# pydata/sparse

Hardware: AMD Instinct MI355X
Metric: GCXS x dense SpMM throughput (GFLOP/s) (higher is better)
Workload: dtype f32; 1 GPU; GCXS(CSR) 1000000x10000 @ 0.01 (100000000 nnz, int32 idx) in 1 nnz-balanced row block(s) x dense 10000x128 fp32; world_size=1, rows_rank0=1000000, idx_dtype=int32, parallelism=row-block x1, mul_add=fma, nan_warning=deferred, prewarm_products=40, default_settings=NAN_WARNING="sync" (verdict read inside every product), kernel=spmm_tiled (cached block stream)

## Files before the change

sparse_amd/csrc/build.py:

```python
import concurrent.futures as cf
import glob
import os
import shutil
import subprocess
import sys

HERE = os.path.dirname(os.path.abspath(__file__))
PKG = os.path.dirname(HERE)
OUT_DIR = os.path.join(PKG, "_lib")
OBJ_DIR = os.path.join(OUT_DIR, "obj")
LIB = os.path.join(OUT_DIR, "libsparse_amd.so")
ARCH = "gfx950"
CXXFLAGS = [
    f"--offload-arch={ARCH}", "-O3", "-std=c++17", "-fPIC", "-ffp-contract=off",
    "-fno-gpu-rdc", "-Wall", "-Wno-unused-function", "-Wno-unused-variable",
]


def _hipcc():
    for c in (os.environ.get("HIPCC"), shutil.which("hipcc"), "/opt/rocm/bin/hipcc"):
        if c and os.path.exists(c):
            return c
    raise RuntimeError("hipcc not found (need ROCm to build libsparse_amd.so)")


def sources():
    return sorted(glob.glob(os.path.join(HERE, "*.hip")))


def _deps():
    return sorted(glob.glob(os.path.join(HERE, "*.h"))) + sorted(glob.glob(os.path.join(HERE, "*.inc"))) + [
        os.path.join(os.path.dirname(PKG), "include", "sparse_amd.h"), os.path.abspath(__file__)]


def is_stale():
    if not os.path.exists(LIB):
        return True
    t = os.path.getmtime(LIB)
    return any(os.path.getmtime(p) > t for p in sources() + _deps())


def _own_deps(src, obj):
    dep = obj[:-2] + ".d"
    if not os.path.exists(dep):
        return _deps()
    words = open(dep).read().replace("\\\n", " ").split()
    files = [w for w in words[1:] if not w.startswith("/opt/") and not w.startswith("/usr/")]
    if any(not os.path.exists(f) for f in files):
        return _deps()
    return files + [os.path.abspath(__file__)]


NO_SPILL = {"spmm_tiled.hip": "spmm_tiled_kernel"}


def _spills(remarks, needle):
    out, name, sg = [], None, 0
    for ln in remarks.splitlines():
        if "Function Name:" in ln:
            name = ln.split("Function Name:")[1].split()[0]
        elif "SGPRs Spill:" in ln:
            sg = int(ln.split("SGPRs Spill:")[1].split()[0])
        elif "VGPRs Spill:" in ln and name is not None:
            vg = int(ln.split("VGPRs Spill:")[1].split()[0])
            if needle in name and (sg or vg):
                out.append((name, sg, vg))
    return out


def _compile(src, force):
    obj = os.path.join(OBJ_DIR, os.path.basename(src)[:-4] + ".o")
    newest = max(os.path.getmtime(p) for p in [src] + _own_deps(src, obj))
    if not force and os.path.exists(obj) and os.path.getmtime(obj) >= newest:
        return obj, ""
    needle = NO_SPILL.get(os.path.basename(src))
    extra = ["-Rpass-analysis=kernel-resource-usage"] if needle else []
    cmd = [_hipcc(), *CXXFLAGS, *extra, "-MD", "-MF", obj[:-2] + ".d", "-c", src, "-o", obj]
    r = subprocess.run(cmd, capture_output=True, text=True)
    if r.returncode != 0:
        raise RuntimeError(f"hipcc failed for {src}:\n{' '.join(cmd)}\n{r.stdout}\n{r.stderr}")
    if needle:
        bad = _spills(r.stderr, needle)
        if bad:
            os.remove(obj)
            raise RuntimeError(f"{os.path.basename(src)}: the compiler spilled registers in " +
                               ", ".join(f"{n[:60]} ({s} SGPR, {v} VGPR)" for n, s, v in bad[:4]) +
                               " - refused (see NO_SPILL in sparse_amd/csrc/build.py)")
        return obj, "\n".join(ln for ln in r.stderr.splitlines() if "-Rpass-analysis" not in ln and "remark:" not in ln)
    return obj, r.stderr


def build(force=False, verbose=False, jobs=None):
    if not force and not is_stale():
        return LIB
    os.makedirs(OBJ_DIR, exist_ok=True)
    srcs = sources()
    jobs = jobs or min(len(srcs), os.cpu_count() or 1)
    with cf.ThreadPoolExecutor(max_workers=jobs) as ex:
        results = list(ex.map(lambda s: _compile(s, force), srcs))
    objs = [o for o, _ in results]
    if verbose:
        for _, w in results:
            if w.strip():
                print(w, file=sys.stderr)
    cmd = [_hipcc(), f"--offload-arch={ARCH}", "-shared", "-fPIC", "-o", LIB + ".tmp", *objs]
    r = subprocess.run(cmd, capture_output=True, text=True)
    if r.returncode != 0:
        raise RuntimeError(f"link failed:\n{' '.join(cmd)}\n{r.stdout}\n{r.stderr}")
    os.replace(LIB + ".tmp", LIB)
    return LIB


if __name__ == "__main__":
    p = build(force="--force" in sys.argv, verbose=True)
    print(p)
```

sparse_amd/csrc/spmm_tiled.hip:

```cpp
#include "common.h"
#include "spmm_tiled_asm.inc"
#include <stdlib.h>
#include <mutex>
#include <set>

namespace spamd {

constexpr int TL_RG = TL_ASM_RG;
constexpr int TL_WAVES = TL_ASM_WAVES;
#ifndef SPAMD_TL_EXPERIMENTAL
static_assert(TL_RG == 35 && TL_WAVES == 16, "experimental tiled-SpMM geometry: build with -DSPAMD_TL_EXPERIMENTAL");
#endif
constexpr int TL_KB = TL_ASM_KB;
constexpr int TL_NBUF = 2;
__host__ __device__ constexpr int tl_d0(int lc, int lr) { return ((lc >> 1) << 11) | ((lc & 1) << 9) | (2 + 2 * lr); }
constexpr int TL_BLOCK_INTS = 16;

template <typename T>
struct TlFmt;
template <>
struct TlFmt<float> {
  static constexpr int EPB = 8, PANEL = 128;
  __device__ static void put(int* stream, int64_t entry, int d0, float v) {
    int* b = stream + (entry / EPB) * TL_BLOCK_INTS + (entry % EPB) * 2;
    typedef int int2v __attribute__((ext_vector_type(2)));
    int2v e;
    e.x = d0;
    e.y = __builtin_bit_cast(int, v);
    *reinterpret_cast<int2v*>(b) = e;
  }
};
template <>
struct TlFmt<double> {
  static constexpr int EPB = 5, PANEL = 64;
  __device__ static void put(int* stream, int64_t entry, int d0, double v) {
    int* b = stream + (entry / EPB) * TL_BLOCK_INTS;
    const int slot = (int)(entry % EPB);
    const long long bits = __builtin_bit_cast(long long, v);
    b[slot] = d0;
    if (slot == 0) b[5] = 0;
    *reinterpret_cast<long long*>(b + 6 + 2 * slot) = bits;
  }
};
typedef int tl_srd_t __attribute__((ext_vector_type(4)));
constexpr int TL_TILE = TL_KB * 512;
constexpr int TL_LDS = TL_NBUF * TL_TILE;
constexpr int TL_DMA_PER_TILE = TL_TILE / 16 / (TL_WAVES * 64);
static_assert(TL_LDS <= 160 * 1024 && TL_KB % (2 * TL_WAVES) == 0 && TL_DMA_PER_TILE == TL_ASM_DMA_PER_TILE,
              "tile geometry is baked into gen_tiled_asm.py");
constexpr int TL_SLACK_BLOCKS = 68;

#define GRID_STRIDE(i, n)                                                          \
  for (int64_t i = (int64_t)blockIdx.x * blockDim.x + threadIdx.x; i < (n);        \
       i += (int64_t)gridDim.x * blockDim.x)

__global__ void __launch_bounds__(256) tl_keys_kernel(const int64_t* __restrict__ rc_keys, int64_t nnz, int64_t K,
                                                      int64_t ntiles, int64_t* __restrict__ out) {
  GRID_STRIDE(i, nnz) {
    const int64_t k = rc_keys[i];
    const int64_t row = k / K, col = k - row * K;
    const int64_t g = row / TL_RG, lr = row - g * TL_RG, t = col / TL_KB, lc = col - t * TL_KB;
    out[i] = ((g * ntiles + t) * TL_RG + lr) * TL_KB + lc;
  }
}

__global__ void __launch_bounds__(256) tl_seg_start_kernel(const int64_t* __restrict__ keys, int64_t nnz,
                                                           int64_t nseg, int64_t* __restrict__ seg_start) {
  GRID_STRIDE(i, nnz + 1) {
    const int64_t hi = i < nnz ? keys[i] / (TL_RG * TL_KB) : nseg;
    const int64_t lo = i > 0 ? keys[i - 1] / (TL_RG * TL_KB) + 1 : 0;
    for (int64_t s = lo; s <= hi; ++s) seg_start[s] = i;
  }
}

__global__ void __launch_bounds__(256) tl_blocks_kernel(const int64_t* __restrict__ seg_start, int64_t nseg, int epb,
                                                        int64_t* __restrict__ nblk) {
  GRID_STRIDE(s, nseg + 1) {
    nblk[s] = s < nseg ? (seg_start[s + 1] - seg_start[s] + epb - 1) / epb : 0;
  }
}

template <typename T>
__global__ void __launch_bounds__(256) tl_pack_kernel(const int64_t* __restrict__ keys, const T* __restrict__ vals,
                                                      int64_t nnz, const int64_t* __restrict__ seg_start,
                                                      const int64_t* __restrict__ blk_off, int* __restrict__ stream) {
  GRID_STRIDE(i, nnz) {
    const int64_t k = keys[i];
    const int64_t lc = k % TL_KB, r1 = k / TL_KB, lr = r1 % TL_RG, s = r1 / TL_RG;
    const int64_t dst = blk_off[s] * TlFmt<T>::EPB + (i - seg_start[s]);
    TlFmt<T>::put(stream, dst, tl_d0((int)lc, (int)lr), vals[i]);
  }
}

constexpr int TL_DIRECT_MAX_TILES = 256;

template <typename I>
__device__ __forceinline__ int tl_row_of(const int64_t* rs, int64_t e) {
  static_assert(TL_RG <= 128, "seven bisection steps");
  int lo = 0, hi = TL_RG;
#pragma unroll
  for (int it = 0; it < (TL_RG <= 64 ? 6 : 7); ++it) {
    const int mid = (lo + hi) >> 1;
    if (hi - lo > 1) {
      if (rs[mid] <= e) lo = mid; else hi = mid;
    }
  }
  return lo;
}

template <typename I>
__global__ void __launch_bounds__(256) tl_count_kernel(int64_t M, int ntiles, int epb, const I* __restrict__ indices,
                                                       const I* __restrict__ indptr, int64_t* __restrict__ nblk,
                                                       int* __restrict__ flags) {
  __shared__ int cnt[TL_DIRECT_MAX_TILES];
  __shared__ int64_t rs[TL_RG + 1];
  const int tid = threadIdx.x;
  const int64_t r0 = (int64_t)blockIdx.x * TL_RG;
  if (tid <= TL_RG) {
    const int64_t r = r0 + tid;
    rs[tid] = (int64_t)indptr[r < M ? r : M];
  }
  for (int t = tid; t < ntiles; t += 256) cnt[t] = 0;
  __syncthreads();
  const int64_t e0 = rs[0], e1 = rs[TL_RG];
  bool bad = false;
  for (int64_t e = e0 + tid; e < e1; e += 256) {
    const int64_t c = (int64_t)indices[e];
    atomicAdd(&cnt[(int)(c / TL_KB)], 1);
    if (e > e0 && (int64_t)indices[e - 1] > c && rs[tl_row_of<I>(rs, e)] != e) bad = true;
  }
  if (bad) flags[0] = 1;
  __syncthreads();
  for (int t = tid; t < ntiles; t += 256) nblk[(int64_t)blockIdx.x * ntiles + t] = (cnt[t] + epb - 1) / epb;
}

template <typename I, typename T>
__global__ void __launch_bounds__(256) tl_fill_kernel(int64_t M, int ntiles, const T* __restrict__ vals,
                                                      const I* __restrict__ indices, const I* __restrict__ indptr,
                                                      const int64_t* __restrict__ blk_off, int* __restrict__ stream) {
  extern __shared__ int tl_fill_lds[];
  __shared__ int64_t rs[TL_RG + 1];
  int* const before = tl_fill_lds;
  int* const runstart = before + TL_RG * ntiles;
  const int tid = threadIdx.x;
  const int64_t r0 = (int64_t)blockIdx.x * TL_RG;
  if (tid <= TL_RG) {
    const int64_t r = r0 + tid;
    rs[tid] = (int64_t)indptr[r < M ? r : M];
  }
  for (int i = tid; i < TL_RG * ntiles; i += 256) before[i] = 0;
  __syncthreads();
  const int64_t e0 = rs[0], e1 = rs[TL_RG];
  for (int64_t e = e0 + tid; e < e1; e += 256) {
    const int t = (int)((int64_t)indices[e] / TL_KB);
// ... 23 lines not shown

__host__ __device__ inline int64_t tl_group_first_block(int64_t e0, int64_t g, int64_t ntiles, int64_t epb) {
  return (e0 + g * ntiles * (epb - 1) + epb - 1) / epb;
}

template <typename I, typename T, bool MAPPED>
__global__ void __launch_bounds__(256) tl_inspect_kernel(int64_t M, int ntiles, int64_t groups, const T* __restrict__ vals,
                                                         const I* __restrict__ indices, const I* __restrict__ indptr,
                                                         unsigned long long* __restrict__ state, int* __restrict__ blk_off,
                                                         int* __restrict__ stream, const int* __restrict__ rowmap,
                                                         const int64_t* __restrict__ vstart) {
  extern __shared__ int tl_fill_lds[];
  __shared__ __attribute__((aligned(16))) int64_t rsab[2 * (TL_RG + 1)];
  __shared__ int wtot[5];
  __shared__ int group_bad;
  constexpr int EPB = TlFmt<T>::EPB;
  int* const before = tl_fill_lds;
  int* const runstart = before + TL_RG * ntiles;
  int* const loff = runstart + TL_RG * ntiles;
  const int tid = threadIdx.x;
  const int64_t g = blockIdx.x;
  const int64_t r0 = g * TL_RG;
  if (tid < TL_RG) {
    if constexpr (MAPPED) {
      const int r = rowmap[r0 + tid];
      rsab[2 * (tid)] = r >= 0 ? (int64_t)indptr[r] : 0;
      rsab[2 * (tid) + 1] = r >= 0 ? (int64_t)indptr[r + 1] : 0;
    } else {
      const int64_t r = r0 + tid;
      rsab[2 * (tid)] = (int64_t)indptr[r < M ? r : M];
      rsab[2 * (tid) + 1] = (int64_t)indptr[r + 1 < M ? r + 1 : M];
    }
  }
  for (int i = tid; i < TL_RG * ntiles; i += 256) before[i] = 0;
  if (tid == 0) group_bad = 0;
  __syncthreads();
  const int64_t e0 = MAPPED ? vstart[g] : rsab[2 * (0)], e1 = MAPPED ? vstart[g + 1] : rsab[2 * (TL_RG - 1) + 1];
  bool bad = false;
  constexpr int RPW = (TL_RG + 3) / 4;
  constexpr int TL_PRE = 2;
  const int wv = tid >> 6, lane = tid & 63;
  unsigned cpre[RPW][TL_PRE];
  T vpre[RPW][TL_PRE];
#pragma unroll
  for (int i = 0; i < RPW; ++i) {
    const int lr = wv + 4 * i;
    const int64_t ra = lr < TL_RG ? rsab[2 * (lr)] : 0, rb = lr < TL_RG ? rsab[2 * (lr) + 1] : 0;
#pragma unroll
    for (int p = 0; p < TL_PRE; ++p) {
      const int64_t e = ra + lane + 64 * p;
      cpre[i][p] = e < rb ? (unsigned)indices[e] : 0xffffffffu;
      vpre[i][p] = e < rb ? vals[e] : T(0);
    }
  }
  auto count_one = [&](int lr, int64_t ra, int64_t e, unsigned c, unsigned cp, bool row_start) {
    const int t = (int)(c / (unsigned)TL_KB);
    atomicAdd(&before[lr * ntiles + t], 1);
    if (!row_start && cp > c) bad = true;
    if (row_start || (int)(cp / (unsigned)TL_KB) != t) runstart[lr * ntiles + t] = (int)(e - (MAPPED ? ra : e0));
  };
#pragma unroll
  for (int i = 0; i < RPW; ++i) {
    const int lr = wv + 4 * i;
    if (lr >= TL_RG) break;
    const int64_t ra = rsab[2 * (lr)], rb = rsab[2 * (lr) + 1];
#pragma unroll
    for (int p = 0; p < TL_PRE; ++p) {
      const int64_t e = ra + lane + 64 * p;
      const unsigned c = cpre[i][p];
      unsigned cp = (unsigned)__shfl_up((int)c, 1, 64);
      if (p > 0) {
        const unsigned last = (unsigned)__builtin_amdgcn_readlane((int)cpre[i][p > 0 ? p - 1 : 0], 63);
        if (lane == 0) cp = last;
      }
      if (e < rb) count_one(lr, ra, e, c, cp, p == 0 && lane == 0);
    }
    for (int64_t e = ra + lane + 64 * TL_PRE; e < rb; e += 64)
      count_one(lr, ra, e, (unsigned)indices[e], (unsigned)indices[e - 1], false);
  }
  if (bad) {
    atomicOr(&state[0], 1ull);
    group_bad = 1;
  }
  __syncthreads();
  int nb = 0, cnt_t = 0;
  for (int t = tid; t < ntiles; t += 256) {
    int c[TL_RG];
#pragma unroll
    for (int lr = 0; lr < TL_RG; ++lr) c[lr] = before[lr * ntiles + t];
    int run = 0;
#pragma unroll
    for (int lr = 0; lr < TL_RG; ++lr) {
      before[lr * ntiles + t] = run;
      run += c[lr];
    }
    cnt_t = run;
    nb = (run + EPB - 1) / EPB;
  }
  const int wid = wv;
  int x = nb;
#pragma unroll
  for (int d = 1; d < 64; d <<= 1) {
    const int y = __shfl_up(x, d, 64);
    if (lane >= d) x += y;
  }
  if (lane == 63) wtot[wid] = x;
  __syncthreads();
  int woff = 0;
  for (int w = 0; w < wid; ++w) woff += wtot[w];
  const int gtotal = wtot[0] + wtot[1] + wtot[2] + wtot[3];
  const int my_off = woff + x - nb;
  const int64_t goff = tl_group_first_block(e0, g, ntiles, EPB);
  const int64_t gnext = tl_group_first_block(e1, g + 1, ntiles, EPB);
  if (tid < ntiles) loff[tid] = my_off;
  __syncthreads();
  if (tid < ntiles) blk_off[g * (ntiles + 1) + tid] = (int)(goff + my_off);
  if (tid == 0) blk_off[g * (ntiles + 1) + ntiles] = (int)(goff + gtotal);
  for (int64_t i = (goff + gtotal) * TL_BLOCK_INTS + tid; i < gnext * TL_BLOCK_INTS; i += 256) stream[i] = 0;
  if (group_bad) {
    for (int64_t i = goff * TL_BLOCK_INTS + tid; i < (goff + gtotal) * TL_BLOCK_INTS; i += 256) stream[i] = 0;
    return;
  }
  auto fill_one = [&](int lr, int64_t ra, int64_t e, unsigned c, T v) {
    const int t = (int)(c / (unsigned)TL_KB);
    const int lc = (int)(c - (unsigned)t * (unsigned)TL_KB);
    const int64_t dst = (goff + loff[t]) * EPB + before[lr * ntiles + t] + ((int)(e - (MAPPED ? ra : e0)) - runstart[lr * ntiles + t]);
    TlFmt<T>::put(stream, dst, tl_d0(lc, lr), v);
  };
#pragma unroll
  for (int i = 0; i < RPW; ++i) {
    const int lr = wv + 4 * i;
    if (lr >= TL_RG) break;
    const int64_t ra = rsab[2 * (lr)], rb = rsab[2 * (lr) + 1];
#pragma unroll
    for (int p = 0; p < TL_PRE; ++p) {
      const int64_t e = ra + lane + 64 * p;
      if (e < rb) fill_one(lr, ra, e, cpre[i][p], vpre[i][p]);
    }
    for (int64_t e = ra + lane + 64 * TL_PRE; e < rb; e += 64) fill_one(lr, ra, e, (unsigned)indices[e], vals[e]);
  }
  if (tid < ntiles) {
    const int64_t first = (goff + my_off) * EPB;
    for (int i = cnt_t; i < nb * EPB; ++i) TlFmt<T>::put(stream, first + i, 0, T(0));
  }
}

__device__ __forceinline__ void tl_dma16(unsigned lds_base, const void* src) {
  asm volatile("s_mov_b32 m0, %0\n\ts_nop 0\n\tglobal_load_lds_dwordx4 %1, off"
               :
               : "s"(lds_base), "v"(src)
               : "memory", "m0");
}

template <int MODE>
__device__ __forceinline__ void tl_phases(const int* stream, int t0, int te, int o0, int o1, int o2, int offreg, int obase,
                                          int ntiles, int nfull, int toff, int mask, unsigned m0wave,
                                          unsigned row_step, int voff, tl_srd_t srd, unsigned& soff) {
  const int lane = threadIdx.x & 63;
  const unsigned blo = (unsigned)((uintptr_t)stream & 0xffffffffu), bhi = (unsigned)((uintptr_t)stream >> 32);
  const int lane8 = lane * 8;
#define TL_PHASES_OPERANDS                                                                                        \
  [soff] "+s"(soff)                                                                                               \
  : [blo] "s"(blo), [bhi] "s"(bhi), [t0] "s"(t0), [te] "s"(te), [o0] "s"(o0), [o1] "s"(o1), [o2] "s"(o2),         \
    [obase] "s"(obase), [ntiles] "s"(ntiles), [nfull] "s"(nfull), [m0wave] "s"(m0wave), [step] "s"(row_step),      \
    [toff] "v"(toff), [lane8] "v"(lane8), [mask] "v"(mask), [offreg] "v"(offreg), [voff] "v"(voff), [srd] "s"(srd)  \
  : "memory", "m0", "scc", "vcc", TL_CLOB_SGPR, TL_CLOB_TMP, TL_CLOB_ACC
  if (MODE == 6)
    asm volatile(TL_ASM_PHASES_I32 : TL_PHASES_OPERANDS);
  else if (MODE == 4)
    asm volatile(TL_ASM_PHASES_F64 : TL_PHASES_OPERANDS);
  else if (MODE == 5)
    asm volatile(TL_ASM_PHASES_F64_EXACT : TL_PHASES_OPERANDS);
  else if (MODE == 3)
    asm volatile(TL_ASM_PHASES_EXACT : TL_PHASES_OPERANDS);
  else if (MODE == 1)
    asm volatile(TL_ASM_PHASES_NOFMA : TL_PHASES_OPERANDS);
  else if (MODE == 2)
    asm volatile(TL_ASM_PHASES_NOLDS : TL_PHASES_OPERANDS);
  else
    asm volatile(TL_ASM_PHASES : TL_PHASES_OPERANDS);
#undef TL_PHASES_OPERANDS
}

__device__ __forceinline__ void tl_block_map(unsigned L, int npanels, int nblocks, int& bx, int& by) {
  const unsigned pin = npanels > 1 ? 2u : 1u;
  const unsigned per_chunk = (unsigned)((nblocks + 7) / 8) * 8u * pin;
  const unsigned chunk = L / per_chunk, l = L % per_chunk;
  const unsigned seq = l >> 3;
  by = uniform((int)(chunk * pin + seq % pin));
  bx = uniform((int)((seq / pin) * 8u + (l & 7u)));
}

template <int DBG, int MODE, typename T>
__global__ void __launch_bounds__(TL_WAVES * 64) __attribute__((amdgpu_num_vgpr(TL_ASM_COMP)))
spmm_tiled_kernel(int64_t M, int64_t K, int ntiles, int touch_lines, const int* __restrict__ stream,
                  const int* __restrict__ blk_off, const T* __restrict__ b, int64_t ldb,
                  T* __restrict__ out, int64_t ldo, int last_cols, int npanels, int nblocks, const int* __restrict__ rowmap) {
  constexpr int PANEL = TlFmt<T>::PANEL;
  constexpr int CPL = PANEL / 64;
  extern __shared__ __attribute__((aligned(16))) char lds[];
  const int tid = threadIdx.x;
  const int lane = tid & 63;
  const int wv = uniform(tid >> 6);
  int bx, by;
  tl_block_map(blockIdx.x, npanels, nblocks, bx, by);
  if (bx >= nblocks || by >= npanels) return;
  const int g = bx * TL_WAVES + wv;
  b += (int64_t)by * PANEL;
  out += (int64_t)by * PANEL;

  asm volatile(TL_ASM_ZERO ::: "memory", TL_CLOB_ACC);

  const int nfull = DBG == 2 ? 0 : (int)(K / TL_KB);
  const unsigned row_step = (unsigned)((2 * TL_WAVES) * ldb * (int64_t)sizeof(T));
  const unsigned m0wave = (unsigned)wv * 2048u;
  const uint64_t bbase = (uint64_t)(uintptr_t)b;
  tl_srd_t srd;
  srd[0] = (int)(bbase & 0xffffffffu);
  srd[1] = (int)((bbase >> 32) & 0xffffu);
  srd[2] = (int)0xffffffffu;
  srd[3] = 0x00020000;
  const int voff = (int)((int64_t)(tid >> 5) * ldb * (int64_t)sizeof(T)) + (tid & 31) * 16;
  unsigned soff = 0;
  auto issue_partial = [&](int t) {
#pragma unroll
    for (int i = 0; i < TL_DMA_PER_TILE; ++i) {
      const int e = (i * (TL_WAVES * 64) + tid) * 16;
      int64_t r = (int64_t)t * TL_KB + (e >> 9);
      if (r >= K) r = K - 1;
      tl_dma16(((unsigned)(i * TL_WAVES + wv) * 2u + (unsigned)(t & 1)) * 1024u,
               reinterpret_cast<const char*>(b + r * ldb) + (e & 511));
    }
  };
  const bool has_partial = DBG != 2 && (int64_t)nfull * TL_KB < K;

  if (nfull > 0)
    asm volatile(TL_ASM_TILE0 : [soff] "+s"(soff) : [m0wave] "s"(m0wave), [step] "s"(row_step), [voff] "v"(voff), [srd] "s"(srd) : "memory", "m0", "scc", "vcc", "s89");
  else if (has_partial)
    issue_partial(0);
  asm volatile("s_waitcnt vmcnt(0)" ::: "memory");
  __syncthreads();

  const int* const myoff = blk_off + (int64_t)g * (ntiles + (touch_lines >> 16));
  touch_lines &= 0xffff;
  const int toff = (lane < touch_lines ? lane : touch_lines - 1) * 64;
  int t = 0;
  while (t < ntiles) {
    const int obase = t;
    const int q = obase + lane;
    int offreg = myoff[q < ntiles ? q : ntiles];
    asm volatile("" : "+v"(offreg));
    int te = obase + 61 < ntiles ? obase + 61 : ntiles;
    if (has_partial && t < nfull - 1 && nfull - 1 < te) te = nfull - 1;
    if (has_partial && t == nfull - 1) issue_partial(nfull);
    auto o = [&](int tt) { return wave_bcast(offreg, (tt < ntiles ? tt : ntiles) - obase); };
    const int o0 = o(t), o1 = o(t + 1), o2 = o(t + 2);
    if (t == 0) {
      const int n = o2 - o0, l = lane < n ? lane : 0;
      asm volatile("global_load_dword " TL_ASM_TOUCH ", %0, off" ::"v"(reinterpret_cast<const char*>(stream + (int64_t)o0 * 16) + l * 64)
                   : "memory", TL_ASM_TOUCH);
    }
    tl_phases<MODE>(stream, t, te, o0, o1, o2, offreg, obase, ntiles, nfull, toff, (int)0xfffffe00, m0wave, row_step, voff, srd, soff);
    t = te;
  }
  asm volatile("s_waitcnt vmcnt(0) lgkmcnt(0)" ::: "memory");

  const int64_t row0 = (int64_t)g * TL_RG;
  const int64_t left = M - row0;
  const int nvalid = left <= 0 ? 0 : (left < TL_RG ? (int)left : TL_RG);
  T* const obase_p = out + row0 * ldo + lane * CPL;
  const int64_t stride_bytes = ldo * (int64_t)sizeof(T);
  int bx2, by2;
  tl_block_map(blockIdx.x, npanels, nblocks, bx2, by2);
  const int ncols = (last_cols > 0 && by2 == npanels - 1) ? last_cols : PANEL;
  if (rowmap) {
    const int* const rm = rowmap + (int64_t)g * TL_RG;
    T* const base_p = out + lane * CPL;
    if (lane * CPL + CPL <= ncols)
      asm volatile(TL_ASM_STORE_PERM
                   :
                   : [lo] "v"((unsigned)((uintptr_t)base_p & 0xffffffffu)), [hi] "v"((unsigned)((uintptr_t)base_p >> 32)),
                     [stride] "s"((unsigned)stride_bytes), [rm] "s"(rm)
                   : "memory", "scc", TL_CLOB_SGPR, TL_CLOB_TMP, TL_CLOB_ACC);
    if constexpr (CPL == 2) {
      if (lane * CPL + 1 == ncols)
        asm volatile(TL_ASM_STORE1_PERM
                     :
                     : [lo] "v"((unsigned)((uintptr_t)base_p & 0xffffffffu)), [hi] "v"((unsigned)((uintptr_t)base_p >> 32)),
                       [stride] "s"((unsigned)stride_bytes), [rm] "s"(rm)
                     : "memory", "scc", TL_CLOB_SGPR, TL_CLOB_TMP);
    }
    return;
  }
  if (lane * CPL + CPL <= ncols)
    asm volatile(TL_ASM_STORE
                 :
                 : [lo] "v"((unsigned)((uintptr_t)obase_p & 0xffffffffu)), [hi] "v"((unsigned)((uintptr_t)obase_p >> 32)),
                   [stride] "s"(stride_bytes), [n] "s"(nvalid)
                 : "memory", "scc", "s36", TL_ASM_BASE, TL_ASM_TOUCH, TL_CLOB_ACC);
  if constexpr (CPL == 2) {
    if (lane * CPL + 1 == ncols)
      asm volatile(TL_ASM_STORE1
                   :
                   : [lo] "v"((unsigned)((uintptr_t)obase_p & 0xffffffffu)), [hi] "v"((unsigned)((uintptr_t)obase_p >> 32)),
                     [stride] "s"(stride_bytes), [n] "s"(nvalid)
                   : "memory", "scc", "s36", TL_ASM_BASE, TL_ASM_TOUCH);
  }
}

static int64_t tl_grid_groups(int64_t M) { return ceil_div(ceil_div(M, (int64_t)TL_RG), (int64_t)TL_WAVES) * TL_WAVES; }

}

using namespace spamd;

static int tl_epb(int val_dtype) { return val_dtype == SPAMD_F32 ? TlFmt<float>::EPB : (val_dtype == SPAMD_F64 ? TlFmt<double>::EPB : 0); }

extern "C" int spamd_spmm_tiled_params(int val_dtype, int* rows_per_group, int* tile_rows, int* groups_per_block,
                                       int* entries_per_block, int* slack_blocks, int* direct_max_tiles,
                                       int* panel_cols) {
  if (!tl_epb(val_dtype)) return SPAMD_ETYPE;
  if (direct_max_tiles) *direct_max_tiles = TL_DIRECT_MAX_TILES;
  if (rows_per_group) *rows_per_group = TL_RG;
  if (tile_rows) *tile_rows = TL_KB;
  if (groups_per_block) *groups_per_block = TL_WAVES;
  if (entries_per_block) *entries_per_block = tl_epb(val_dtype);
  if (slack_blocks) *slack_blocks = TL_SLACK_BLOCKS;
  if (panel_cols) *panel_cols = val_dtype == SPAMD_F32 ? TlFmt<float>::PANEL : TlFmt<double>::PANEL;
  return 0;
}

static unsigned tl_blocks_for(int64_t n) {
  int64_t blocks = ceil_div(n, (int64_t)256);
  if (blocks > 8192) blocks = 8192;
  if (blocks < 1) blocks = 1;
  return (unsigned)blocks;
}

extern "C" int spamd_spmm_tiled_keys(int64_t nnz, const int64_t* rowcol_keys, int64_t K, int64_t* tiled_keys,
                                     void* stream) {
  if (nnz < 0 || K <= 0) return SPAMD_EINVAL;
  if (nnz == 0) return 0;
  hipLaunchKernelGGL(tl_keys_kernel, dim3(tl_blocks_for(nnz)), dim3(256), 0, (hipStream_t)stream, rowcol_keys, nnz, K,
                     ceil_div(K, (int64_t)TL_KB), tiled_keys);
  return launch_status();
}

extern "C" int spamd_spmm_tiled_lists(int val_dtype, int64_t nnz, const int64_t* tiled_keys_sorted, int64_t M, int64_t K,
                                      int64_t* seg_start, int64_t* nblk, void* stream) {
  if (nnz < 0 || M < 0 || K <= 0) return SPAMD_EINVAL;
  if (!tl_epb(val_dtype)) return SPAMD_ETYPE;
  const int64_t nseg = tl_grid_groups(M) * ceil_div(K, (int64_t)TL_KB);
  hipLaunchKernelGGL(tl_seg_start_kernel, dim3(tl_blocks_for(nnz + 1)), dim3(256), 0, (hipStream_t)stream,
                     tiled_keys_sorted, nnz, nseg, seg_start);
  hipLaunchKernelGGL(tl_blocks_kernel, dim3(tl_blocks_for(nseg + 1)), dim3(256), 0, (hipStream_t)stream, seg_start,
                     nseg, tl_epb(val_dtype), nblk);
  return launch_status();
}

static int tl_clear_blocks(int64_t total_blocks, int* blocks, hipStream_t s) {
  return (int)hipMemsetAsync(blocks, 0, (size_t)(total_blocks + TL_SLACK_BLOCKS) * TL_BLOCK_INTS * sizeof(int), s);
}

extern "C" int spamd_spmm_tiled_pack(int val_dtype, int64_t nnz, const int64_t* tiled_keys_sorted, const void* vals_sorted,
                                     const int64_t* seg_start, const int64_t* blk_off, int64_t total_blocks,
                                     int* blocks, void* stream) {
  if (nnz < 0 || total_blocks < 0) return SPAMD_EINVAL;
  if (!tl_epb(val_dtype)) return SPAMD_ETYPE;
  int rc = tl_clear_blocks(total_blocks, blocks, (hipStream_t)stream);
  if (rc) return rc;
  if (nnz == 0) return 0;
  if (val_dtype == SPAMD_F32)
    hipLaunchKernelGGL(tl_pack_kernel<float>, dim3(tl_blocks_for(nnz)), dim3(256), 0, (hipStream_t)stream, tiled_keys_sorted,
                       (const float*)vals_sorted, nnz, seg_start, blk_off, blocks);
  else
    hipLaunchKernelGGL(tl_pack_kernel<double>, dim3(tl_blocks_for(nnz)), dim3(256), 0, (hipStream_t)stream, tiled_keys_sorted,
                       (const double*)vals_sorted, nnz, seg_start, blk_off, blocks);
  return launch_status();
}

extern "C" int spamd_spmm_tiled_count(int val_dtype, int idx_dtype, int64_t M, int64_t K, const void* a_indices,
                                      const void* a_indptr, int64_t* nblk, int* flags, void* stream) {
  if (M < 0 || K <= 0) return SPAMD_EINVAL;
  if (!tl_epb(val_dtype)) return SPAMD_ETYPE;
  const int64_t ntiles = ceil_div(K, (int64_t)TL_KB);
  if (ntiles > TL_DIRECT_MAX_TILES) return SPAMD_EINVAL;
  const int64_t groups = tl_grid_groups(M);
  hipError_t e = hipMemsetAsync(flags, 0, sizeof(int), (hipStream_t)stream);
  if (e != hipSuccess) return (int)e;
  e = hipMemsetAsync(nblk + groups * ntiles, 0, sizeof(int64_t), (hipStream_t)stream);
  if (e != hipSuccess) return (int)e;
  if (groups == 0) return 0;
  SPAMD_DISPATCH_IDX(idx_dtype, I, hipLaunchKernelGGL(tl_count_kernel<I>, dim3((unsigned)groups), dim3(256), 0,
                                                    (hipStream_t)stream, M, (int)ntiles, tl_epb(val_dtype),
                                                    (const I*)a_indices, (const I*)a_indptr, nblk, flags))
  return launch_status();
}

template <typename I, typename T>
static int tl_launch_fill(int64_t M, int64_t ntiles, const T* a_data, const I* a_indices, const I* a_indptr,
                          const int64_t* blk_off, int* blocks, hipStream_t s) {
  const int lds = (int)(2 * TL_RG * ntiles * sizeof(int));
  auto kern = &tl_fill_kernel<I, T>;
  if (lds > 48 * 1024) {
    hipError_t e = hipFuncSetAttribute(reinterpret_cast<const void*>(kern), hipFuncAttributeMaxDynamicSharedMemorySize, lds);
    if (e != hipSuccess) return (int)e;
  }
  hipLaunchKernelGGL(kern, dim3((unsigned)tl_grid_groups(M)), dim3(256), lds, s, M, (int)ntiles, a_data, a_indices, a_indptr,
                     blk_off, blocks);
  return launch_status();
}

extern "C" int spamd_spmm_tiled_fill(int val_dtype, int idx_dtype, int64_t M, int64_t K, const void* a_data,
                                     const void* a_indices, const void* a_indptr, const int64_t* blk_off,
                                     int64_t total_blocks, int* blocks, void* stream) {
  if (M < 0 || K <= 0 || total_blocks < 0) return SPAMD_EINVAL;
  if (!tl_epb(val_dtype)) return SPAMD_ETYPE;
  const int64_t ntiles = ceil_div(K, (int64_t)TL_KB);
  if (ntiles > TL_DIRECT_MAX_TILES) return SPAMD_EINVAL;
  int rc = tl_clear_blocks(total_blocks, blocks, (hipStream_t)stream);
  if (rc) return rc;
  if (tl_grid_groups(M) == 0) return 0;
  SPAMD_DISPATCH_IDX(idx_dtype, I, {
    if (val_dtype == SPAMD_F32)
      return tl_launch_fill<I, float>(M, ntiles, (const float*)a_data, (const I*)a_indices, (const I*)a_indptr, blk_off,
                                      blocks, (hipStream_t)stream);
    return tl_launch_fill<I, double>(M, ntiles, (const double*)a_data, (const I*)a_indices, (const I*)a_indptr, blk_off,
                                     blocks, (hipStream_t)stream);
  })
  return SPAMD_ETYPE;
}

template <typename I, typename T>
static int tl_launch_inspect(int64_t M, int64_t ntiles, const T* a_data, const I* a_indices, const I* a_indptr,
                             unsigned long long* state, int* blk_off, int* blocks, hipStream_t s, int64_t map_groups = 0,
                             const int* rowmap = nullptr, const int64_t* vstart = nullptr) {
  const int64_t groups = rowmap ? map_groups : tl_grid_groups(M);
  const int lds = (int)((2 * TL_RG * ntiles + ntiles + 1) * sizeof(int));
  auto kern = rowmap ? &tl_inspect_kernel<I, T, true> : &tl_inspect_kernel<I, T, false>;
  if (lds > 48 * 1024) {
    hipError_t e = hipFuncSetAttribute(reinterpret_cast<const void*>(kern), hipFuncAttributeMaxDynamicSharedMemorySize, lds);
    if (e != hipSuccess) return (int)e;
  }
  hipLaunchKernelGGL(kern, dim3((unsigned)groups), dim3(256), lds, s, M, (int)ntiles, groups, a_data, a_indices, a_indptr,
                     state, blk_off, blocks, rowmap, vstart);
  return launch_status();
}

constexpr int TL_MAP_CLASSES = 6;
__host__ __device__ inline int tl_map_slots(int c) { return c == 5 ? TL_RG : (1 << c); }
__host__ __device__ inline int tl_map_class(int64_t len, int64_t cap) {
  return len > cap / 2 ? 0 : (len > cap / 4 ? 1 : (len > cap / 8 ? 2 : (len > cap / 16 ? 3 : (len > cap / 32 ? 4 : 5))));
}

template <typename I>
__global__ void __launch_bounds__(256) tl_map_stats_kernel(int64_t M, int64_t cap, int64_t maxlen, const I* __restrict__ indptr,
                                                           int64_t* __restrict__ keys, int* __restrict__ rows,
                                                           unsigned long long* __restrict__ stats) {
  __shared__ unsigned cnt[TL_MAP_CLASSES];
  if (threadIdx.x < TL_MAP_CLASSES) cnt[threadIdx.x] = 0;
// ... 682 lines not shown
    if (!padded && tid < GPB) {
      const int c = tbase[tid], nb = (c + EPB - 1) / EPB;
      const int64_t first = (goff_s[tid] + lo16[tid]) * EPB;
      for (int q = c; q < nb * EPB; ++q) TlFmt<T>::put(stream, first + q, 0, T(0));
    }
    __syncthreads();
  }
}

template <typename I, typename T>
static int tl_launch_inspect_csc(int64_t M, int64_t K, int64_t ntiles, const T* a_data, const I* a_indices, const I* a_indptr,
                                 int* ws, unsigned long long* state, int* blk_off, int* blocks, hipStream_t s) {
  const int64_t groups = tl_grid_groups(M);
  const int64_t nblocks = groups / TL_WAVES;
  if (nblocks >= ((int64_t)1 << 31)) return SPAMD_EINVAL;
  const bool hist = groups <= TL_CSC_HIST_GROUPS;
  int* const split = ws;
  int* const cnt = split + (nblocks + 1) * K;
  int* const rel = cnt + TL_CSC_HIST_PARTS * groups * ntiles;
  const int64_t words = ((nblocks + 1) * K + TL_CSC_HIST_PARTS * groups * ntiles + groups * (ntiles + 1) + 1) & ~(int64_t)1;
  unsigned long long* const look = reinterpret_cast<unsigned long long*>(ws + words);
  long long* const e0 = reinterpret_cast<long long*>(look) + groups;
  const int64_t owgs = ceil_div(groups, (int64_t)64);
  const int nlook = (int)(owgs + 2);
  static_assert(TL_WAVES >= 3, "groups (a multiple of TL_WAVES) >= ceil(groups / 64) + 2");
  if (!hist) {
    const unsigned sgrid = (unsigned)std::min<int64_t>(K, (int64_t)256 * 64);
    hipLaunchKernelGGL((tl_csc_split_kernel<I>), dim3(sgrid), dim3(256), 0, s, M, K, nblocks, a_indices, a_indptr, split, state, look, nlook);
  }
  const dim3 grid((unsigned)nblocks, (unsigned)ceil_div(ntiles, (int64_t)TL_CSC_TC));
  if (hist) {
    auto hk = &tl_csc_hist_kernel<I>;
    const int lds = (int)((groups + 1) / 2 * sizeof(int));
    if (lds > 48 * 1024) {
      hipError_t e = hipFuncSetAttribute(reinterpret_cast<const void*>(hk), hipFuncAttributeMaxDynamicSharedMemorySize, lds);
      if (e != hipSuccess) return (int)e;
    }
    hipLaunchKernelGGL(hk, dim3((unsigned)ntiles, TL_CSC_HIST_PARTS), dim3(1024), lds, s, M, K, (int)ntiles, groups, nblocks,
                       a_indices, a_indptr, cnt, split, state, look, nlook);
  } else {
    hipLaunchKernelGGL((tl_csc_count_kernel<I>), grid, dim3(256), 0, s, K, (int)ntiles, nblocks, groups, a_indices, a_indptr, (const int*)split,
                       (const unsigned long long*)state, cnt);
  }
  if (hist)
    hipLaunchKernelGGL((tl_csc_offsets_kernel<TlFmt<T>::EPB, TL_CSC_HIST_PARTS>), dim3((unsigned)owgs), dim3(64), 0, s,
                       groups, (int)ntiles, (const int*)cnt, (const unsigned long long*)state, rel, look, e0);
  else
    hipLaunchKernelGGL((tl_csc_offsets_kernel<TlFmt<T>::EPB, 1>), dim3((unsigned)owgs), dim3(64), 0, s,
                       groups, (int)ntiles, (const int*)cnt, (const unsigned long long*)state, rel, look, e0);
  const int64_t fgrid = 8 * ceil_div(nblocks, (int64_t)8) * ceil_div(ntiles, (int64_t)TL_CSC_TC);
  if (fgrid >= ((int64_t)1 << 31)) return SPAMD_EINVAL;
  hipLaunchKernelGGL((tl_csc_fill_kernel<I, T>), dim3((unsigned)fgrid), dim3(256), 0, s, K, (int)ntiles, a_data, a_indices,
                     a_indptr, (const int*)split, (const unsigned long long*)state, (const int*)rel, (const long long*)e0, nblocks,
                     blk_off, blocks);
  return launch_status();
}

extern "C" int64_t spamd_spmm_tiled_inspect_csc_ws(int64_t M, int64_t K) {
  if (M < 0 || K <= 0) return -1;
  const int64_t ntiles = ceil_div(K, (int64_t)TL_KB), groups = tl_grid_groups(M), nblocks = groups / TL_WAVES;
  return (nblocks + 1) * K + TL_CSC_HIST_PARTS * groups * ntiles + groups * (ntiles + 1) + 2 + 2 * (2 * groups + 1) + 16;
}

extern "C" int spamd_spmm_tiled_inspect_csc(int val_dtype, int idx_dtype, int64_t M, int64_t K, const void* a_data,
                                            const void* a_indices, const void* a_indptr, int* ws, void* state, int* blk_off,
                                            int* blocks, void* stream) {
  if (M < 0 || K <= 0) return SPAMD_EINVAL;
  if (!tl_epb(val_dtype)) return SPAMD_ETYPE;
  if ((uintptr_t)ws % 8) return SPAMD_EINVAL;
  const int64_t ntiles = ceil_div(K, (int64_t)TL_KB);
  if (ntiles > TL_DIRECT_MAX_TILES) return SPAMD_EINVAL;
  hipError_t e = hipMemsetAsync(state, 0, sizeof(unsigned long long), (hipStream_t)stream);
  if (e != hipSuccess) return (int)e;
  if (tl_grid_groups(M) == 0) return 0;
  SPAMD_DISPATCH_IDX(idx_dtype, I, {
    if (val_dtype == SPAMD_F32)
      return tl_launch_inspect_csc<I, float>(M, K, ntiles, (const float*)a_data, (const I*)a_indices, (const I*)a_indptr, ws,
                                             (unsigned long long*)state, blk_off, blocks, (hipStream_t)stream);
    return tl_launch_inspect_csc<I, double>(M, K, ntiles, (const double*)a_data, (const I*)a_indices, (const I*)a_indptr, ws,
                                            (unsigned long long*)state, blk_off, blocks, (hipStream_t)stream);
  })
  return SPAMD_ETYPE;
}

static int tl_set_lds_once(const void* kern) { return set_max_dynamic_lds(kern, TL_LDS); }

template <typename T, typename KERN>
static int tl_launch(KERN kern, int64_t M, int64_t K, int64_t N, const int* blocks, const int* blk_off, const T* b,
                     int64_t ldb, T* out, int64_t ldo, int touch_lines, bool group_ends, int last_cols, hipStream_t s,
                     const int* rowmap = nullptr, int64_t map_groups = 0) {
  if (int rc = tl_set_lds_once(reinterpret_cast<const void*>(kern))) return rc;
  const int64_t blocks_n = (rowmap ? map_groups : tl_grid_groups(M)) / TL_WAVES;
  const int64_t npanels = N / TlFmt<T>::PANEL;
  const int64_t grid = ceil_div(blocks_n, (int64_t)8) * 8 * (npanels > 1 ? ceil_div(npanels, (int64_t)2) * 2 : 1);
  if (grid >= ((int64_t)1 << 31) || blocks_n >= ((int64_t)1 << 31)) return SPAMD_EINVAL;
  hipLaunchKernelGGL(kern, dim3((unsigned)grid), dim3(TL_WAVES * 64), TL_LDS, s, M, K,
                     (int)ceil_div(K, (int64_t)TL_KB), touch_lines | (group_ends ? 1 << 16 : 0), blocks, blk_off, b, ldb, out, ldo,
                     last_cols, (int)npanels, (int)blocks_n, rowmap);
  return launch_status();
}

static int tl_product(int val_dtype, int64_t M, int64_t K, int64_t N, const int* blocks, const int* blk_off, const void* b,
                      int64_t ldb, void* out, int64_t ldo, unsigned flags, void* stream, const int* rowmap, int64_t map_groups);

extern "C" int spamd_spmm_tiled(int val_dtype, int64_t M, int64_t K, int64_t N, const int* blocks, const int* blk_off,
                                const void* b, int64_t ldb, void* out, int64_t ldo, unsigned flags, void* stream) {
  return tl_product(val_dtype, M, K, N, blocks, blk_off, b, ldb, out, ldo, flags, stream, nullptr, 0);
}

extern "C" int spamd_spmm_tiled_mapped(int val_dtype, int64_t M, int64_t groups, int64_t K, int64_t N, const int* blocks,
                                       const int* blk_off, const int* rowmap, const void* b, int64_t ldb, void* out, int64_t ldo,
                                       unsigned flags, void* stream) {
  if (!rowmap || groups <= 0 || groups % TL_WAVES) return SPAMD_EINVAL;
  if (ldo * (val_dtype == SPAMD_F32 ? 4 : 8) >= ((int64_t)1 << 32)) return SPAMD_EINVAL;
  return tl_product(val_dtype, M, K, N, blocks, blk_off, b, ldb, out, ldo, flags | SPAMD_TILED_GROUP_ENDS, stream, rowmap, groups);
}

static int tl_product(int val_dtype, int64_t M, int64_t K, int64_t N, const int* blocks, const int* blk_off, const void* b,
                      int64_t ldb, void* out, int64_t ldo, unsigned flags, void* stream, const int* rowmap, int64_t map_groups) {
  if (!tl_epb(val_dtype)) return SPAMD_ETYPE;
  const int panel = val_dtype == SPAMD_F32 ? TlFmt<float>::PANEL : TlFmt<double>::PANEL;
  const int esz = val_dtype == SPAMD_F32 ? 4 : 8;
  if (M < 0 || K <= 0 || N <= 0 || N % panel != 0 || N / panel > 65535 || K / TL_KB >= ((int64_t)1 << 30)) return SPAMD_EINVAL;
  if (M == 0) return 0;
  if (((uintptr_t)b % 16) || ((ldb * esz) % 16) || ((uintptr_t)out % esz) || ((uintptr_t)blocks % 64))
    return SPAMD_EINVAL;
  if ((K + 2 * TL_KB) * ldb * esz >= ((int64_t)1 << 32)) return SPAMD_EINVAL;
  hipStream_t s = (hipStream_t)stream;
  const bool exact = (flags & SPAMD_EXACT_MULADD) != 0;
  const bool ends = (flags & SPAMD_TILED_GROUP_ENDS) != 0;
  const bool i32 = (flags & SPAMD_TILED_INT32) != 0;
  if (i32 && val_dtype != SPAMD_F32) return SPAMD_EINVAL;
  const int last_cols = (int)((flags >> 16) & 0xffu);
  if (last_cols > panel) return SPAMD_EINVAL;
  if (ldo < N - panel + (last_cols ? last_cols : panel)) return SPAMD_EINVAL;
  int touch = (int)((flags >> 8) & 0xffu);
  if (touch == 0) touch = 12;
  if (touch > 64) touch = 64;
  if (val_dtype == SPAMD_F64) {
    const double* bb = (const double*)b;
    double* oo = (double*)out;
    return exact ? tl_launch<double>(&spmm_tiled_kernel<0, 5, double>, M, K, N, blocks, blk_off, bb, ldb, oo, ldo, touch, ends, last_cols, s, rowmap, map_groups)
                 : tl_launch<double>(&spmm_tiled_kernel<0, 4, double>, M, K, N, blocks, blk_off, bb, ldb, oo, ldo, touch, ends, last_cols, s, rowmap, map_groups);
  }
  const float* bb = (const float*)b;
  float* oo = (float*)out;
#ifdef SPAMD_TUNING
  const char* dbg_env = getenv("SPAMD_TILED_DBG");
  const int dbg = dbg_env ? atoi(dbg_env) : 0;
  if (dbg == 2) return tl_launch<float>(&spmm_tiled_kernel<2, 0, float>, M, K, N, blocks, blk_off, bb, ldb, oo, ldo, touch, ends, last_cols, s, rowmap, map_groups);
  if (dbg == 5) return tl_launch<float>(&spmm_tiled_kernel<0, 1, float>, M, K, N, blocks, blk_off, bb, ldb, oo, ldo, touch, ends, last_cols, s, rowmap, map_groups);
  if (dbg == 6) return tl_launch<float>(&spmm_tiled_kernel<0, 2, float>, M, K, N, blocks, blk_off, bb, ldb, oo, ldo, touch, ends, last_cols, s, rowmap, map_groups);
  if (dbg == 7) return tl_launch<float>(&spmm_tiled_kernel<2, 2, float>, M, K, N, blocks, blk_off, bb, ldb, oo, ldo, touch, ends, last_cols, s, rowmap, map_groups);
#endif
  if (i32) return tl_launch<float>(&spmm_tiled_kernel<0, 6, float>, M, K, N, blocks, blk_off, bb, ldb, oo, ldo, touch, ends, last_cols, s, rowmap, map_groups);
  return exact ? tl_launch<float>(&spmm_tiled_kernel<0, 3, float>, M, K, N, blocks, blk_off, bb, ldb, oo, ldo, touch, ends, last_cols, s, rowmap, map_groups)
               : tl_launch<float>(&spmm_tiled_kernel<0, 0, float>, M, K, N, blocks, blk_off, bb, ldb, oo, ldo, touch, ends, last_cols, s, rowmap, map_groups);
}
```

Before: 30240 GFLOP/s.

## Switch tiled SpMM to generated ring asm with lane-parked scalar state

Replaces the hand-written phase asm include with a generated ring-buffer variant and parks per-wave scalar loop state (tile bounds, offsets, stream base, counts) in lanes of one VGPR, so the inner asm no longer needs them as SGPR operands. Epilogue values (M, ldo, out, rowmap, block mapping) are reloaded from the kernarg segment after the main loop instead of being kept live across it. The aim is to free SGPRs and VGPRs for a deeper LDS ring or more in-flight loads. In exchange it adds readlane/writelane overhead, a build-time generator step, and a stricter spill check. A tuning-only stall-stamping mode is also added.

```diff
diff --git a/sparse_amd/csrc/build.py b/sparse_amd/csrc/build.py
--- a/sparse_amd/csrc/build.py
+++ b/sparse_amd/csrc/build.py
@@ -28,9 +28,21 @@
     return sorted(glob.glob(os.path.join(HERE, "*.hip")))
 
 
+GEN_TILED = os.path.join(os.path.dirname(PKG), "tools", "gen_tiled_asm.py")
+GEN_TILED_INC = os.path.join(HERE, "spmm_tiled_ring_asm.inc")
+
+
+def _generate():
+    if os.path.exists(GEN_TILED_INC) and os.path.getmtime(GEN_TILED_INC) >= os.path.getmtime(GEN_TILED):
+        return
+    r = subprocess.run([sys.executable, GEN_TILED], capture_output=True, text=True)
+    if r.returncode != 0 or not os.path.exists(GEN_TILED_INC):
+        raise RuntimeError(f"{GEN_TILED} failed:\n{r.stdout}\n{r.stderr}")
+
+
 def _deps():
     return sorted(glob.glob(os.path.join(HERE, "*.h"))) + sorted(glob.glob(os.path.join(HERE, "*.inc"))) + [
-        os.path.join(os.path.dirname(PKG), "include", "sparse_amd.h"), os.path.abspath(__file__)]
+        os.path.join(os.path.dirname(PKG), "include", "sparse_amd.h"), os.path.abspath(__file__), GEN_TILED]
 
 
 def is_stale():
@@ -80,6 +92,11 @@
     if r.returncode != 0:
         raise RuntimeError(f"hipcc failed for {src}:\n{' '.join(cmd)}\n{r.stdout}\n{r.stderr}")
     if needle:
+        seen = [ln for ln in r.stderr.splitlines() if "Function Name:" in ln and needle in ln]
+        if not seen or "SGPRs Spill:" not in r.stderr or "VGPRs Spill:" not in r.stderr:
+            os.remove(obj)
+            raise RuntimeError(f"{os.path.basename(src)}: no kernel-resource-usage remark for {needle}* - the spill check "
+                               "cannot be made (see NO_SPILL in sparse_amd/csrc/build.py)")
         bad = _spills(r.stderr, needle)
         if bad:
             os.remove(obj)
@@ -91,8 +108,9 @@
 
 
 def build(force=False, verbose=False, jobs=None):
-    if not force and not is_stale():
+    if not force and os.path.exists(GEN_TILED_INC) and not is_stale():
         return LIB
+    _generate()
     os.makedirs(OBJ_DIR, exist_ok=True)
     srcs = sources()
     jobs = jobs or min(len(srcs), os.cpu_count() or 1)
diff --git a/sparse_amd/csrc/spmm_tiled.hip b/sparse_amd/csrc/spmm_tiled.hip
--- a/sparse_amd/csrc/spmm_tiled.hip
+++ b/sparse_amd/csrc/spmm_tiled.hip
@@ -1,5 +1,5 @@
 #include "common.h"
-#include "spmm_tiled_asm.inc"
+#include "spmm_tiled_ring_asm.inc"
 #include <stdlib.h>
 #include <mutex>
 #include <set>
@@ -329,19 +329,44 @@
                : "memory", "m0");
 }
 
+#define TL_STR2(x) #x
+#define TL_STR(x) TL_STR2(x)
+__device__ __forceinline__ int tl_park_fixed(const int* stream, int ntiles, int nfull, unsigned m0wave) {
+  const unsigned blo = (unsigned)((uintptr_t)stream & 0xffffffffu), bhi = (unsigned)((uintptr_t)stream >> 32);
+  int park = 0;
+  asm volatile("v_writelane_b32 %0, %1, " TL_STR(TL_PARK_NTILES) "\n\tv_writelane_b32 %0, %2, " TL_STR(TL_PARK_NFULL)
+               "\n\tv_writelane_b32 %0, %3, " TL_STR(TL_PARK_M0WAVE) "\n\tv_writelane_b32 %0, %4, " TL_STR(TL_PARK_BLO)
+               "\n\tv_writelane_b32 %0, %5, " TL_STR(TL_PARK_BHI)
+               : "+v"(park)
+               : "s"(ntiles), "s"(nfull), "s"(m0wave), "s"(blo), "s"(bhi));
+  return park;
+}
+
 template <int MODE>
-__device__ __forceinline__ void tl_phases(const int* stream, int t0, int te, int o0, int o1, int o2, int offreg, int obase,
-                                          int ntiles, int nfull, int toff, int mask, unsigned m0wave,
-                                          unsigned row_step, int voff, tl_srd_t srd, unsigned& soff) {
+__device__ __forceinline__ void tl_phases(int& park, int t0, int te, int o0, int o1, int o2, int offreg, int obase, int toff,
+                                          int mask, unsigned row_step, int voff, tl_srd_t srd, unsigned& soff) {
   const int lane = threadIdx.x & 63;
-  const unsigned blo = (unsigned)((uintptr_t)stream & 0xffffffffu), bhi = (unsigned)((uintptr_t)stream >> 32);
   const int lane8 = lane * 8;
+  asm volatile("v_writelane_b32 %0, %1, " TL_STR(TL_PARK_T0) "\n\tv_writelane_b32 %0, %2, " TL_STR(TL_PARK_TE)
+               "\n\tv_writelane_b32 %0, %3, " TL_STR(TL_PARK_O0) "\n\tv_writelane_b32 %0, %4, " TL_STR(TL_PARK_O1)
+               "\n\tv_writelane_b32 %0, %5, " TL_STR(TL_PARK_O2) "\n\tv_writelane_b32 %0, %6, " TL_STR(TL_PARK_OBASE)
+               : "+v"(park)
+               : "s"(t0), "s"(te), "s"(o0), "s"(o1), "s"(o2), "s"(obase));
 #define TL_PHASES_OPERANDS                                                                                        \
   [soff] "+s"(soff)                                                                                               \
-  : [blo] "s"(blo), [bhi] "s"(bhi), [t0] "s"(t0), [te] "s"(te), [o0] "s"(o0), [o1] "s"(o1), [o2] "s"(o2),         \
-    [obase] "s"(obase), [ntiles] "s"(ntiles), [nfull] "s"(nfull), [m0wave] "s"(m0wave), [step] "s"(row_step),      \
+  : [step] "s"(row_step), [park] "v"(park),                                                                       \
     [toff] "v"(toff), [lane8] "v"(lane8), [mask] "v"(mask), [offreg] "v"(offreg), [voff] "v"(voff), [srd] "s"(srd)  \
   : "memory", "m0", "scc", "vcc", TL_CLOB_SGPR, TL_CLOB_TMP, TL_CLOB_ACC
+#ifdef SPAMD_TUNING
+  if (MODE == 7) {
+    asm volatile(TL_ASM_PHASES_STAMP
+                 : [soff] "+s"(soff), [park] "+v"(park)
+                 : [step] "s"(row_step), [toff] "v"(toff), [lane8] "v"(lane8), [mask] "v"(mask), [offreg] "v"(offreg),
+                   [voff] "v"(voff), [srd] "s"(srd)
+                 : "memory", "m0", "scc", "vcc", TL_CLOB_SGPR, TL_CLOB_TMP, TL_CLOB_ACC);
+    return;
+  }
+#endif
   if (MODE == 6)
     asm volatile(TL_ASM_PHASES_I32 : TL_PHASES_OPERANDS);
   else if (MODE == 4)
@@ -367,6 +392,21 @@
   by = uniform((int)(chunk * pin + seq % pin));
   bx = uniform((int)((seq / pin) * 8u + (l & 7u)));
 }
+
+template <typename T>
+struct TlKernArgs {
+  int64_t M, K;
+  int ntiles, touch_lines;
+  const int* stream;
+  const int* blk_off;
+  const T* b;
+  int64_t ldb;
+  T* out;
+  int64_t ldo;
+  int last_cols, npanels, nblocks;
+  const int* rowmap;
+};
+static_assert(offsetof(TlKernArgs<float>, last_cols) == 72 && offsetof(TlKernArgs<float>, rowmap) == 88, "kernel-argument layout");
 
 template <int DBG, int MODE, typename T>
 __global__ void __launch_bounds__(TL_WAVES * 64) __attribute__((amdgpu_num_vgpr(TL_ASM_COMP)))
@@ -412,7 +452,7 @@
   const bool has_partial = DBG != 2 && (int64_t)nfull * TL_KB < K;
 
   if (nfull > 0)
-    asm volatile(TL_ASM_TILE0 : [soff] "+s"(soff) : [m0wave] "s"(m0wave), [step] "s"(row_step), [voff] "v"(voff), [srd] "s"(srd) : "memory", "m0", "scc", "vcc", "s89");
+    asm volatile(TL_ASM_TILE0 : [soff] "+s"(soff) : [m0wave] "s"(m0wave), [step] "s"(row_step), [voff] "v"(voff), [srd] "s"(srd) : "memory", "m0", "scc", "vcc", TL_ASM_LDSDST);
   else if (has_partial)
     issue_partial(0);
   asm volatile("s_waitcnt vmcnt(0)" ::: "memory");
@@ -421,6 +461,7 @@
   const int* const myoff = blk_off + (int64_t)g * (ntiles + (touch_lines >> 16));
   touch_lines &= 0xffff;
   const int toff = (lane < touch_lines ? lane : touch_lines - 1) * 64;
+  int park = tl_park_fixed(stream, ntiles, nfull, m0wave);
   int t = 0;
   while (t < ntiles) {
     const int obase = t;
@@ -437,21 +478,27 @@
       asm volatile("global_load_dword " TL_ASM_TOUCH ", %0, off" ::"v"(reinterpret_cast<const char*>(stream + (int64_t)o0 * 16) + l * 64)
                    : "memory", TL_ASM_TOUCH);
     }
-    tl_phases<MODE>(stream, t, te, o0, o1, o2, offreg, obase, ntiles, nfull, toff, (int)0xfffffe00, m0wave, row_step, voff, srd, soff);
+    tl_phases<MODE>(park, t, te, o0, o1, o2, offreg, obase, toff, (int)0xfffffe00, row_step, voff, srd, soff);
     t = te;
   }
   asm volatile("s_waitcnt vmcnt(0) lgkmcnt(0)" ::: "memory");
 
-  const int64_t row0 = (int64_t)g * TL_RG;
+  typedef const TlKernArgs<T> __attribute__((address_space(4))) * ka_ptr_t;
+  ka_ptr_t ka = (ka_ptr_t)__builtin_amdgcn_kernarg_segment_ptr();
+  asm volatile("" : "+s"(ka));
+  M = ka->M, ldo = ka->ldo, last_cols = ka->last_cols, npanels = ka->npanels, nblocks = ka->nblocks, rowmap = ka->rowmap;
+  int bx2, by2;
+  tl_block_map(blockIdx.x, npanels, nblocks, bx2, by2);
+  out = ka->out + (int64_t)by2 * PANEL;
+  const int g2 = bx2 * TL_WAVES + uniform((int)(threadIdx.x >> 6));
+  const int64_t row0 = (int64_t)g2 * TL_RG;
   const int64_t left = M - row0;
   const int nvalid = left <= 0 ? 0 : (left < TL_RG ? (int)left : TL_RG);
   T* const obase_p = out + row0 * ldo + lane * CPL;
   const int64_t stride_bytes = ldo * (int64_t)sizeof(T);
-  int bx2, by2;
-  tl_block_map(blockIdx.x, npanels, nblocks, bx2, by2);
   const int ncols = (last_cols > 0 && by2 == npanels - 1) ? last_cols : PANEL;
   if (rowmap) {
-    const int* const rm = rowmap + (int64_t)g * TL_RG;
+    const int* const rm = rowmap + (int64_t)g2 * TL_RG;
     T* const base_p = out + lane * CPL;
     if (lane * CPL + CPL <= ncols)
       asm volatile(TL_ASM_STORE_PERM
@@ -483,6 +530,14 @@
                      [stride] "s"(stride_bytes), [n] "s"(nvalid)
                    : "memory", "scc", "s36", TL_ASM_BASE, TL_ASM_TOUCH);
   }
+#ifdef SPAMD_TUNING
+  if constexpr (MODE == 7) {
+    if (lane == 0 && nvalid > 0) {
+      unsigned* const w = reinterpret_cast<unsigned*>(out + row0 * ldo);
+      w[0] = (unsigned)__builtin_amdgcn_readlane(park, TL_PARK_STALL), w[1] = (unsigned)__builtin_amdgcn_readlane(park, TL_PARK_TOTAL);
+    }
+  }
+#endif
 }
 
 static int64_t tl_grid_groups(int64_t M) { return ceil_div(ceil_div(M, (int64_t)TL_RG), (int64_t)TL_WAVES) * TL_WAVES; }
@@ -1471,6 +1526,7 @@
   if (dbg == 5) return tl_launch<float>(&spmm_tiled_kernel<0, 1, float>, M, K, N, blocks, blk_off, bb, ldb, oo, ldo, touch, ends, last_cols, s, rowmap, map_groups);
   if (dbg == 6) return tl_launch<float>(&spmm_tiled_kernel<0, 2, float>, M, K, N, blocks, blk_off, bb, ldb, oo, ldo, touch, ends, last_cols, s, rowmap, map_groups);
   if (dbg == 7) return tl_launch<float>(&spmm_tiled_kernel<2, 2, float>, M, K, N, blocks, blk_off, bb, ldb, oo, ldo, touch, ends, last_cols, s, rowmap, map_groups);
+  if (dbg == 8) return tl_launch<float>(&spmm_tiled_kernel<0, 7, float>, M, K, N, blocks, blk_off, bb, ldb, oo, ldo, touch, ends, last_cols, s, rowmap, map_groups);
 #endif
   if (i32) return tl_launch<float>(&spmm_tiled_kernel<0, 6, float>, M, K, N, blocks, blk_off, bb, ldb, oo, ldo, touch, ends, last_cols, s, rowmap, map_groups);
   return exact ? tl_launch<float>(&spmm_tiled_kernel<0, 3, float>, M, K, N, blocks, blk_off, bb, ldb, oo, ldo, touch, ends, last_cols, s, rowmap, map_groups)
```

Result: slower. 29630 GFLOP/s (-2.0%).
